# facebookresearch/multipathnet

Hardware: NVIDIA H100
Metric: proposals/sec (higher is better)
Workload: dtype fp32 (wgmma split emulation, fp32 accumulate: 3 bf16 products per MAC, 2 fp16 products in fc6/fc7)

## Files before the change

multipathnet_b200/csrc/gemm_tc.cu:

```cuda
#include "conv_gemm.cuh"
#include "wgmma.cuh"
#include "fp8_e4m3.cuh"
#include <algorithm>
#include <stdlib.h>
#include <string.h>

namespace {

constexpr int BM = 128;
constexpr int BK = 64;
constexpr int TC_THREADS = 384;
constexpr int CONS_THREADS = 256;
constexpr int A_TILE_BYTES = BM * BK * 2;
constexpr int SMEM_BUDGET = 196608;

__host__ __device__ constexpr int a_planes(OperandScheme ops) { return (ops == OperandScheme::BF16X1 || ops == OperandScheme::FP8X1) ? 1 : 2; }
__host__ __device__ constexpr int b_planes(OperandScheme ops) { return ops == OperandScheme::BF16X3 ? 2 : 1; }
__host__ __device__ constexpr int elem_bytes(OperandScheme ops) { return ops == OperandScheme::FP8X1 ? 1 : 2; }
__host__ __device__ constexpr int row_bytes(int BN, OperandScheme ops) { return (ops == OperandScheme::FP8X1 || BN == 256) ? 64 : 128; }
__host__ __device__ constexpr int stage_k(int BN, OperandScheme ops) { return row_bytes(BN, ops) / elem_bytes(ops); }
__host__ __device__ constexpr int kb_steps(int BN, OperandScheme ops) { return BK / stage_k(BN, ops); }
__host__ __device__ constexpr int a_tile_bytes(int BN, OperandScheme ops) { return BM * row_bytes(BN, ops); }
__host__ __device__ constexpr int stage_bytes(int BN, OperandScheme ops = OperandScheme::BF16X3) {
  return (a_planes(ops) * BM + b_planes(ops) * BN) * row_bytes(BN, ops);
}
__host__ __device__ constexpr int max_stages(int BN, OperandScheme ops) { return row_bytes(BN, ops) == 64 ? 8 : 4; }
__host__ __device__ constexpr int num_stages(int BN, OperandScheme ops = OperandScheme::BF16X3) {
  return (SMEM_BUDGET / stage_bytes(BN, ops)) > max_stages(BN, ops) ? max_stages(BN, ops) : (SMEM_BUDGET / stage_bytes(BN, ops));
}
constexpr int EPI_WARP_BYTES = 16 * 128;
constexpr int EPI_BYTES = (CONS_THREADS / 32) * EPI_WARP_BYTES;
__host__ __device__ constexpr int tc_smem_bytes(int BN, OperandScheme ops) {
  return num_stages(BN, ops) * stage_bytes(BN, ops) + EPI_BYTES + 1024  + 256 ;
}

struct TcParams {
  int N, Ho, Wo, Cout;
  int kh, kw, stride, pad;
  int cblocks;
  int tn, th, tw;
  int tiles_img, tiles_h, tiles_w, tiles_n;
  int units;
  const float *bias;
  const __nv_bfloat16 *res_hi, *res_lo; long long res_ld;
  __nv_bfloat16 *out_hi, *out_lo; long long out_ld;
  float *out_f32; long long out_f32_ld;
  __nv_bfloat16 *pool_hi, *pool_lo; long long pool_ld; int Hp, Wp;
  int relu;
  int splitk, kb_per_split;
  long long split_stride;
  unsigned long long *tl_min, *tl_max;
  float acc_scale;
  int out_fmt;
  unsigned *ovf;
  const int *a_exp, *b_exp; long long sample_pix;
};

__device__ __forceinline__ unsigned long long gtimer() {
  unsigned long long t; asm volatile("mov.u64 %0, %%globaltimer;" : "=l"(t)); return t;
}
__device__ __forceinline__ void tl_min_stamp(const unsigned long long *base_, int i) {
  if (base_) atomicMin(const_cast<unsigned long long *>(base_) + i, gtimer());
}
__device__ __forceinline__ void tl_max_stamp(const unsigned long long *base_, int i) {
  if (base_) atomicMax(const_cast<unsigned long long *>(base_) + i, gtimer());
}
__device__ __forceinline__ uint32_t smem_u32(const void *p) { return (uint32_t)__cvta_generic_to_shared(p); }
__device__ __forceinline__ void mbar_init(uint32_t bar, uint32_t count) {
  asm volatile("mbarrier.init.shared::cta.b64 [%0], %1;" ::"r"(bar), "r"(count) : "memory");
}
__device__ __forceinline__ void mbar_expect_tx(uint32_t bar, uint32_t bytes) {
  asm volatile("mbarrier.arrive.expect_tx.shared::cta.b64 _, [%0], %1;" ::"r"(bar), "r"(bytes) : "memory");
}
__device__ __forceinline__ void mbar_arrive(uint32_t bar) {
  asm volatile("mbarrier.arrive.shared::cta.b64 _, [%0];" ::"r"(bar) : "memory");
}
__device__ __forceinline__ void mbar_wait(uint32_t bar, uint32_t parity) {
  uint32_t done;
  uint32_t spins = 0;
  do {
    asm volatile(
        "{\n\t.reg .pred p;\n\t"
        "mbarrier.try_wait.parity.shared::cta.b64 p, [%1], %2;\n\t"
        "selp.u32 %0, 1, 0, p;\n\t}"
        : "=r"(done) : "r"(bar), "r"(parity) : "memory");
    if (!done && ++spins == (1u << 26)) __trap();
  } while (!done);
}
__device__ __forceinline__ void tma_load_4d(uint32_t dst, const CUtensorMap *tm, uint32_t bar, int c0, int c1,
                                            int c2, int c3) {
  asm volatile(
      "cp.async.bulk.tensor.4d.shared::cluster.global.mbarrier::complete_tx::bytes [%0], [%1, {%3, %4, %5, %6}], [%2];"
      ::"r"(dst), "l"(reinterpret_cast<uint64_t>(tm)), "r"(bar), "r"(c0), "r"(c1), "r"(c2), "r"(c3) : "memory");
}
__device__ __forceinline__ void tma_load_2d(uint32_t dst, const CUtensorMap *tm, uint32_t bar, int c0, int c1) {
  asm volatile(
      "cp.async.bulk.tensor.2d.shared::cluster.global.mbarrier::complete_tx::bytes [%0], [%1, {%3, %4}], [%2];"
      ::"r"(dst), "l"(reinterpret_cast<uint64_t>(tm)), "r"(bar), "r"(c0), "r"(c1) : "memory");
}
__device__ __forceinline__ void prefetch_tmap(const CUtensorMap *tm) {
  asm volatile("prefetch.tensormap [%0];" ::"l"(reinterpret_cast<uint64_t>(tm)) : "memory");
}

__device__ __forceinline__ uint64_t make_smem_desc(uint32_t saddr) {
  uint64_t d = 0;
  d |= (uint64_t)((saddr & 0x3FFFFu) >> 4);
  d |= (uint64_t)1 << 16;
  d |= (uint64_t)(1024 >> 4) << 32;
  d |= (uint64_t)1 << 62;
  return d;
}

__device__ __forceinline__ uint64_t make_smem_desc_64b(uint32_t saddr) {
  uint64_t d = 0;
  d |= (uint64_t)((saddr & 0x3FFFFu) >> 4);
  d |= (uint64_t)1 << 16;
// ... 97 lines not shown
      float b[2] = {0.f, 0.f};
      int eb[2] = {0, 0};
#pragma unroll
      for (int k = 0; k < 2; ++k) {
        if (p.bias && c + k < p.Cout) b[k] = __ldg(p.bias + c + k);
        if constexpr (OPS == OperandScheme::FP8X1) eb[k] = __ldg(p.b_exp + c + k);
      }
#pragma unroll
      for (int i = 0; i < 2; ++i) {
        float &f0 = f[4 * j + 2 * i], &f1 = f[4 * j + 2 * i + 1];
        if constexpr (OPS == OperandScheme::FP16X2) { f0 *= p.acc_scale; f1 *= p.acc_scale; }
        if constexpr (OPS == OperandScheme::FP8X1) {
          f0 *= mpn_fp8::pow2(-(ea[i] + eb[0])); f1 *= mpn_fp8::pow2(-(ea[i] + eb[1]));
        }
        if (p.bias) {
          if (c < p.Cout) f0 += b[0];
          if (c + 1 < p.Cout) f1 += b[1];
        }
        if (p.res_hi && full8 && fok[i]) {
          const float2 x = bf16x2_to_float2(*reinterpret_cast<const uint32_t *>(p.res_hi + fpix[i] * p.res_ld + c));
          const float2 y = bf16x2_to_float2(*reinterpret_cast<const uint32_t *>(p.res_lo + fpix[i] * p.res_ld + c));
          f0 += x.x + y.x; f1 += x.y + y.y;
        }
        if (p.relu) { f0 = fmaxf(f0, 0.f); f1 = fmaxf(f1, 0.f); }
        if (out_f32 && fok[i]) {
          float *o = out_f32 + fpix[i] * p.out_f32_ld + c;
          if (c < p.Cout) o[0] = f0;
          if (c + 1 < p.Cout) o[1] = f1;
        }
      }
    }
    float mx[16];
    if (pool) {
#pragma unroll
      for (int j = 0; j < 8; ++j)
#pragma unroll
        for (int k = 0; k < 2; ++k) {
          float top = fok[0] ? f[4 * j + k] : -INFINITY, bot = fok[1] ? f[4 * j + 2 + k] : -INFINITY;
          top = fmaxf(top, __shfl_xor_sync(0xffffffffu, top, 4));
          bot = fmaxf(bot, __shfl_xor_sync(0xffffffffu, bot, 4));
          mx[2 * j + k] = fmaxf(top, bot);
        }
    }
#pragma unroll 1
    for (int plane = 0; plane < 2; ++plane) {
      if (p.out_hi) {
        uint32_t v[16];
#pragma unroll
        for (int j = 0; j < 8; ++j)
#pragma unroll
          for (int i = 0; i < 2; ++i) {
            uint32_t hi2 = 0, lo2 = 0;
            if (fok[i]) split_x2(p.out_fmt, f[4 * j + 2 * i], f[4 * j + 2 * i + 1], hi2, lo2, p.ovf);
            v[8 * i + j] = plane ? lo2 : hi2;
          }
        store_plane_chunk(so, v, plane ? p.out_lo : p.out_hi, p.out_ld, p, u, rbase, col0, lane);
      }
      if (pool) {
        const int pr = lane >> 3;
        __syncwarp();
        if (!(lane & 4) && fok[0]) {
#pragma unroll
          for (int j = 0; j < 8; ++j) {
            uint32_t hi2, lo2;
            split_x2(p.out_fmt, mx[2 * j], mx[2 * j + 1], hi2, lo2, p.ovf);
            const uint32_t a = so + (uint32_t)(pr * 128 + ((j ^ pr) * 16) + 4 * (lane & 3));
            asm volatile("st.shared.b32 [%0], %1;" ::"r"(a), "r"(plane ? lo2 : hi2) : "memory");
          }
        }
        __syncwarp();
        const int ch = lane & 7;
        uint4 d;
        asm volatile("ld.shared.v4.b32 {%0, %1, %2, %3}, [%4];" : "=r"(d.x), "=r"(d.y), "=r"(d.z), "=r"(d.w)
                     : "r"(so + (uint32_t)(pr * 128 + ((ch ^ pr) * 16))) : "memory");
        if (pok && col0 + 8 * ch < p.Cout)
          *reinterpret_cast<uint4 *>((plane ? p.pool_lo : p.pool_hi) + ppix * p.pool_ld + col0 + 8 * ch) = d;
      }
    }
#pragma unroll
    for (int k = 0; k + 32 < BN / 2; ++k) acc[k] = acc[k + 32];
  }
}

template <int BN, OperandScheme OPS = OperandScheme::BF16X3>
__global__ void __launch_bounds__(TC_THREADS, 1)
conv_gemm_tc_kernel(const __grid_constant__ CUtensorMap tmA_hi, const __grid_constant__ CUtensorMap tmA_lo,
                    const __grid_constant__ CUtensorMap tmB_hi, const __grid_constant__ CUtensorMap tmB_lo,
                    const TcParams p) {
  constexpr int S = num_stages(BN, OPS);
  constexpr int STAGE = stage_bytes(BN, OPS);
  constexpr int A_TILE = a_tile_bytes(BN, OPS);
  constexpr int B_TILE_BYTES = BN * row_bytes(BN, OPS);
  constexpr int B_OFF = a_planes(OPS) * A_TILE;
  constexpr int KSTEPS = kb_steps(BN, OPS);
  static_assert(S >= 2 && 2 * S * 8 <= 256, "ring depth: at least two stages, barriers in their 256 bytes");
  extern __shared__ uint8_t smem_raw[];
  uint8_t *smem = reinterpret_cast<uint8_t *>((reinterpret_cast<uintptr_t>(smem_raw) + 1023) & ~(uintptr_t)1023);
  uint64_t *bars = reinterpret_cast<uint64_t *>(smem + (size_t)S * STAGE + EPI_BYTES);
  const uint32_t smem_base = smem_u32(smem);
  const uint32_t bar_base = smem_u32(bars);
  auto full_bar = [&](int s) { return bar_base + 8u * s; };
  auto empty_bar = [&](int s) { return bar_base + 8u * (S + s); };

  const int tid = threadIdx.x, lane = tid & 31;
  const int num_kb = p.kh * p.kw * p.cblocks;

  if (tid == 0) {
    tl_min_stamp(p.tl_min, 0);
    if (a_planes(OPS) == 1) { prefetch_tmap(&tmA_hi); prefetch_tmap(&tmB_hi); }
    else { prefetch_tmap(&tmA_hi); prefetch_tmap(&tmA_lo); prefetch_tmap(&tmB_hi); prefetch_tmap(&tmB_lo); }
    for (int s = 0; s < S; ++s) { mbar_init(full_bar(s), 1); mbar_init(empty_bar(s), CONS_THREADS / 32); }
    asm volatile("fence.mbarrier_init.release.cluster;" ::: "memory");
  }
  __syncthreads();
  asm volatile("griddepcontrol.wait;" ::: "memory");
  asm volatile("griddepcontrol.launch_dependents;" ::: "memory");
  if (tid == 0) tl_min_stamp(p.tl_min, 1);

  if (tid < 128) {
    asm volatile("setmaxnreg.dec.sync.aligned.u32 24;" ::: "memory");
    if (tid == 0) {
      int it = 0;
      for (int unit = (int)blockIdx.x; unit < p.units; unit += (int)gridDim.x) {
        const UnitPos u = unit_pos(p, unit);
        const int kb0 = u.split * p.kb_per_split, kb1 = min(num_kb, kb0 + p.kb_per_split);
        const int w_in0 = u.twi * p.tw * p.stride - p.pad, h_in0 = u.thi * p.th * p.stride - p.pad, n0 = u.tni * p.tn;
        const int b_row0 = u.nt * BN;
        for (int kb = kb0; kb < kb1; ++kb) {
          const int tap = kb / p.cblocks, cb = kb - tap * p.cblocks;
          const int khi = tap / p.kw, kwi = tap - khi * p.kw;
#pragma unroll
          for (int h = 0; h < KSTEPS; ++h, ++it) {
            const int s = it % S; const uint32_t ph = (uint32_t)(it / S) & 1u;
            const int ka = cb * BK + h * stage_k(BN, OPS), kk = kb * BK + h * stage_k(BN, OPS);
            mbar_wait(empty_bar(s), ph ^ 1u);
            const uint32_t sa = smem_base + (uint32_t)s * STAGE;
            mbar_expect_tx(full_bar(s), (uint32_t)STAGE);
            tma_load_4d(sa, &tmA_hi, full_bar(s), ka, w_in0 + kwi, h_in0 + khi, n0);
            if (a_planes(OPS) == 2) tma_load_4d(sa + A_TILE, &tmA_lo, full_bar(s), ka, w_in0 + kwi, h_in0 + khi, n0);
            tma_load_2d(sa + B_OFF, &tmB_hi, full_bar(s), kk, b_row0);
            if (b_planes(OPS) == 2) tma_load_2d(sa + B_OFF + B_TILE_BYTES, &tmB_lo, full_bar(s), kk, b_row0);
          }
        }
      }
    }
    return;
  }

  asm volatile("setmaxnreg.inc.sync.aligned.u32 240;" ::: "memory");
  const int e = tid - 128;
  const int g = e >> 7, wq = (e >> 5) & 3;
  const uint32_t so = smem_base + (uint32_t)(S * STAGE + (e >> 5) * EPI_WARP_BYTES);
  int it = 0;
  for (int unit = (int)blockIdx.x; unit < p.units; unit += (int)gridDim.x) {
    const UnitPos u = unit_pos(p, unit);
    const int kb0 = u.split * p.kb_per_split, kb1 = min(num_kb, kb0 + p.kb_per_split);
    float acc[BN / 2];
#pragma unroll
    for (int i = 0; i < BN / 2; ++i) acc[i] = 0.f;
    if constexpr (OPS == OperandScheme::FP8X1) {
      float part[BN / 2];
#pragma unroll
      for (int i = 0; i < BN / 2; ++i) part[i] = 0.f;
      for (int kb = kb0; kb < kb1; ++kb, ++it) {
        const int s = it % S; const uint32_t ph = (uint32_t)(it / S) & 1u;
        mbar_wait(full_bar(s), ph);
        if (it == 0 && e == 0) tl_min_stamp(p.tl_min, 2);
        const uint32_t sa = smem_base + (uint32_t)s * STAGE;
        const uint64_t a8 = make_smem_desc_64b(sa + (uint32_t)g * (A_TILE / 2));
        const uint64_t b8 = make_smem_desc_64b(sa + B_OFF);
#pragma unroll
        for (int k = 0; k < BK / 32; ++k) {
          wgmma_fence_acc(part);
          wgmma_fence();
          wgmma_e4m3_nk32<BN>(part, a8 + (uint64_t)(2 * k), b8 + (uint64_t)(2 * k), 0u);
          wgmma_commit();
          wgmma_wait<0>();
          wgmma_fence_acc(part);
#pragma unroll
          for (int i = 0; i < BN / 2; ++i) acc[i] += part[i];
        }
        if (lane == 0) mbar_arrive(empty_bar(s));
      }
    } else {
      const int steps = (kb1 - kb0) * KSTEPS;
      for (int i = 0; i < steps; ++i, ++it) {
        const int s = it % S; const uint32_t ph = (uint32_t)(it / S) & 1u;
        mbar_wait(full_bar(s), ph);
        if (it == 0 && e == 0) tl_min_stamp(p.tl_min, 2);
        const uint32_t sa = smem_base + (uint32_t)s * STAGE;
        auto desc = [](uint32_t a) { return row_bytes(BN, OPS) == 64 ? make_smem_desc_64b(a) : make_smem_desc(a); };
        const uint64_t a_hi = desc(sa + (uint32_t)g * (A_TILE / 2));
        const uint64_t a_lo = desc(sa + A_TILE + (uint32_t)g * (A_TILE / 2));
        const uint64_t b_hi = desc(sa + B_OFF);
        const uint64_t b_lo = desc(sa + B_OFF + B_TILE_BYTES);
        wgmma_fence_acc(acc);
        wgmma_fence();
        mma_kstep<BN, OPS>(acc, a_hi, a_lo, b_hi, b_lo, i == 0);
        wgmma_commit();
        wgmma_wait<1>();
        wgmma_fence_acc(acc);
        if (i > 0 && lane == 0) mbar_arrive(empty_bar((it - 1) % S));
      }
      wgmma_wait<0>();
      wgmma_fence_acc(acc);
      if (lane == 0) mbar_arrive(empty_bar((it - 1) % S));
    }
    if (e == 0) tl_max_stamp(p.tl_max, 0);
    const uint32_t t_epi = (p.tl_max && e == 0) ? (uint32_t)gtimer() : 0u;
    tile_epilogue<BN, OPS>(p, u, acc, g, wq, lane, so);
    if (e == 0) {
      tl_max_stamp(p.tl_max, 1);
      if (p.tl_max) atomicAdd(p.tl_max + 3, (unsigned long long)((uint32_t)gtimer() - t_epi));
    }
  }
}


constexpr int C1_THREADS = 256;
constexpr int C1_A_BYTES = 2 * A_TILE_BYTES;
constexpr int C1_B_BYTES = 2 * 64 * 128;
constexpr int C1_OUT_WARP = 16 * 128;
constexpr int C1_SMEM = 2 * C1_A_BYTES + C1_B_BYTES + (C1_THREADS / 32) * C1_OUT_WARP + 1024;

__device__ __forceinline__ void conv1_gather(const float *__restrict__ x, int pix, int pixels, int H, int W, int bhalf,
                                             float (&in)[16]) {
#pragma unroll
  for (int k = 0; k < 16; ++k) in[k] = 0.f;
  if (pix < pixels) {
    const int HW = H * W;
    const int n = pix / HW, rem = pix - n * HW;
    const int ho = rem / W, wo = rem - ho * W;
    const float *x0 = x + ((size_t)n * 3 * HW + (size_t)(ho - 1) * W + (wo - 1));
    const bool rok[3] = {ho >= 1, true, ho + 1 < H}, cok[3] = {wo >= 1, true, wo + 1 < W};
#pragma unroll
    for (int k = 0; k < 16; ++k) {
      const int kk = 16 * bhalf + k;
      if (kk < 27) {
        const int ci = kk / 9, r = (kk / 3) % 3, q = kk % 3;
        in[k] = (rok[r] && cok[q]) ? __ldg(x0 + ci * HW + r * W + q) : 0.f;
      }
    }
  }
// ... 97 lines not shown
      for (int h = 0; h < 2; ++h) {
        float &f0 = acc[4 * j + 2 * h], &f1 = acc[4 * j + 2 * h + 1];
        f0 += b.x; f1 += b.y;
        if (relu) { f0 = fmaxf(f0, 0.f); f1 = fmaxf(f1, 0.f); }
      }
    }
    const int pix0 = tile * BM + 64 * g + 16 * (warp & 3);
#pragma unroll 1
    for (int plane = 0; plane < 2; ++plane) {
      uint32_t v[16];
#pragma unroll
      for (int j = 0; j < 8; ++j)
#pragma unroll
        for (int h = 0; h < 2; ++h) {
          uint32_t hi2, lo2;
          split_bf16x2(acc[4 * j + 2 * h], acc[4 * j + 2 * h + 1], hi2, lo2);
          v[8 * h + j] = plane ? lo2 : hi2;
        }
      conv1_store_plane(so, v, plane ? out_lo : out_hi, pix0, pixels, lane);
    }
  }
}

struct ReduceParams {
  const float *ws; long long split_stride; int splitk; long long pixels; int Cout;
  const float *bias; const __nv_bfloat16 *res_hi, *res_lo; long long res_ld; int relu;
  __nv_bfloat16 *out_hi, *out_lo; long long out_ld; float *out_f32; long long out_f32_ld;
  OutScatter scatter;
};
__global__ void __launch_bounds__(256) splitk_reduce_kernel(const ReduceParams r) {
  MPN_PDL_SYNC();
  const long long idx = (long long)blockIdx.x * blockDim.x + threadIdx.x;
  if (idx >= r.pixels * r.Cout) return;
  const long long pix = idx / r.Cout; const int c = (int)(idx - pix * r.Cout);
  float acc = 0.f;
  for (int s = 0; s < r.splitk; ++s) acc += r.ws[(long long)s * r.split_stride + idx];
  if (r.bias) acc += __ldg(r.bias + c);
  if (r.res_hi) acc += join_bf16(r.res_hi[pix * r.res_ld + c], r.res_lo[pix * r.res_ld + c]);
  if (r.relu) acc = fmaxf(acc, 0.f);
  if (r.out_hi) { __nv_bfloat16 h, l; split_bf16(acc, h, l); r.out_hi[pix * r.out_ld + c] = h; r.out_lo[pix * r.out_ld + c] = l; }
  if (r.scatter.n > 0) {
#pragma unroll 1
    for (int g = 0; g < r.scatter.n; ++g)
      if (c >= r.scatter.seg[g].c0 && c < r.scatter.seg[g].c1) { r.scatter.seg[g].ptr[pix * r.scatter.seg[g].ld + (c - r.scatter.seg[g].c0)] = acc; break; }
  } else if (r.out_f32) r.out_f32[pix * r.out_f32_ld + c] = acc;
}

typedef CUresult (*PFN_encodeTiled)(CUtensorMap *, CUtensorMapDataType, cuuint32_t, void *, const cuuint64_t *,
                                    const cuuint64_t *, const cuuint32_t *, const cuuint32_t *, CUtensorMapInterleave,
                                    CUtensorMapSwizzle, CUtensorMapL2promotion, CUtensorMapFloatOOBfill);
PFN_encodeTiled get_encode_fn() {
  static PFN_encodeTiled fn = nullptr;
  if (!fn) {
    void *p = nullptr; cudaDriverEntryPointQueryResult q;
    if (cudaGetDriverEntryPoint("cuTensorMapEncodeTiled", &p, cudaEnableDefault, &q) == cudaSuccess &&
        q == cudaDriverEntryPointSuccess)
      fn = reinterpret_cast<PFN_encodeTiled>(p);
  }
  return fn;
}

int encode_map(mpn_ctx *ctx, CUtensorMap *tm, const void *base, int rank, const cuuint64_t *dims,
               const cuuint64_t *strides_bytes , const cuuint32_t *box, const cuuint32_t *estr, int BN, OperandScheme ops) {
  const bool fp8 = ops == OperandScheme::FP8X1;
  PFN_encodeTiled fn = get_encode_fn();
  if (!fn) return mpn_fail(ctx, MPN_ERR_CUDA, "cuTensorMapEncodeTiled entry point unavailable");
  CUresult r = fn(tm, fp8 ? CU_TENSOR_MAP_DATA_TYPE_UINT8 : CU_TENSOR_MAP_DATA_TYPE_BFLOAT16, (cuuint32_t)rank, const_cast<void *>(base), dims,
                  strides_bytes, box, estr, CU_TENSOR_MAP_INTERLEAVE_NONE, row_bytes(BN, ops) == 64 ? CU_TENSOR_MAP_SWIZZLE_64B : CU_TENSOR_MAP_SWIZZLE_128B,
                  CU_TENSOR_MAP_L2_PROMOTION_L2_256B, CU_TENSOR_MAP_FLOAT_OOB_FILL_NONE);
  if (r != CUDA_SUCCESS) {
    char b[256];
    snprintf(b, sizeof b, "cuTensorMapEncodeTiled failed (%d): rank %d dims %llu %llu box %u %u", (int)r, rank,
             (unsigned long long)dims[0], (unsigned long long)dims[1], box[0], box[1]);
    return mpn_fail(ctx, MPN_ERR_CUDA, b);
  }
  return MPN_OK;
}

inline bool tc_use_pdl() {
  static const int on = [] { const char *e = getenv("MPN_TC_PDL"); return (e && e[0] == '0') ? 0 : 1; }();
  return on != 0;
}

template <int BN, OperandScheme OPS = OperandScheme::BF16X3>
int launch_bn(mpn_ctx *ctx, const ConvPlan &pl, const TcParams &tp) {
  const int smem = tc_smem_bytes(BN, OPS);
  constexpr int bslot = BN == 256 ? 2 : (BN == 128 ? 1 : 0);
  constexpr int slot = OPS == OperandScheme::FP16X2 ? 3 : (OPS == OperandScheme::BF16X1 ? 5 + bslot
                                                         : (OPS == OperandScheme::FP8X1 ? 8 + bslot : bslot));
  if (!ctx->tc_attr_set[slot]) {
    MPN_CUDA(ctx, cudaFuncSetAttribute(conv_gemm_tc_kernel<BN, OPS>, cudaFuncAttributeMaxDynamicSharedMemorySize, smem));
    ctx->tc_attr_set[slot] = 1;
  }
  const long long units = (long long)pl.tiles_img * pl.tiles_h * pl.tiles_w * pl.tiles_n * pl.splitk;
  MPN_CHECK_ARG(ctx, units > 0 && units < (1ll << 31), "conv_tc: grid size out of range");
  TcParams tpu = tp;
  tpu.units = (int)units;
  cudaLaunchConfig_t cfg = {};
  cfg.gridDim = dim3((unsigned)std::min<long long>(units, ctx->sm_count));
  cfg.blockDim = dim3(TC_THREADS); cfg.dynamicSmemBytes = (size_t)smem; cfg.stream = ctx->stream;
  cudaLaunchAttribute attr[1];
  int na = 0;
  if (tc_use_pdl()) {
    attr[na].id = cudaLaunchAttributeProgrammaticStreamSerialization;
    attr[na].val.programmaticStreamSerializationAllowed = 1;
    ++na;
  }
  cfg.attrs = attr; cfg.numAttrs = na;
  MPN_CUDA(ctx, cudaLaunchKernelEx(&cfg, conv_gemm_tc_kernel<BN, OPS>, pl.tmA_hi, pl.tmA_lo, pl.tmB_hi, pl.tmB_lo, tpu));
  MPN_LAUNCHED(ctx);
  return MPN_OK;
}

int launch_ops(mpn_ctx *ctx, const ConvPlan &pl, const TcParams &tp) {
  if (pl.ops == OperandScheme::FP16X2) return launch_bn<256, OperandScheme::FP16X2>(ctx, pl, tp);
  if (pl.ops == OperandScheme::FP8X1)
    return pl.BN == 128 ? launch_bn<128, OperandScheme::FP8X1>(ctx, pl, tp) : launch_bn<64, OperandScheme::FP8X1>(ctx, pl, tp);
  if (pl.ops == OperandScheme::BF16X1) {
    switch (pl.BN) {
      case 256: return launch_bn<256, OperandScheme::BF16X1>(ctx, pl, tp);
      case 128: return launch_bn<128, OperandScheme::BF16X1>(ctx, pl, tp);
      default: return launch_bn<64, OperandScheme::BF16X1>(ctx, pl, tp);
    }
  }
  switch (pl.BN) {
    case 256: return launch_bn<256>(ctx, pl, tp);
    case 128: return launch_bn<128>(ctx, pl, tp);
    default: return launch_bn<64>(ctx, pl, tp);
  }
}

}

int conv1_tc_launch(mpn_ctx *ctx, const float *x_nchw, int N, int H, int W, const float *w_dev, const float *bias_dev, int relu,
                    DTensor &y) {
  MPN_CHECK_ARG(ctx, y.hi && y.lo && y.C == 64 && y.ld % 8 == 0, "conv1_tc: output must be 64-channel split planes");
  MPN_CHECK_ARG(ctx, bias_dev, "conv1_tc: bias missing");
  MPN_CHECK_ARG(ctx, y.ld == 64 && (long long)N * H * W < (1ll << 31) - 256, "conv1_tc: dense 64-channel output and < 2^31 pixels");
  if (!ctx->tc_attr_set[4]) {
    MPN_CUDA(ctx, cudaFuncSetAttribute(conv1_tc_kernel, cudaFuncAttributeMaxDynamicSharedMemorySize, C1_SMEM));
    ctx->tc_attr_set[4] = 1;
  }
  const long long tiles = ((long long)N * H * W + BM - 1) / BM;
  cudaLaunchConfig_t cfg = {};
  cfg.gridDim = dim3((unsigned)std::min<long long>(tiles, 2ll * ctx->sm_count)); cfg.blockDim = dim3(C1_THREADS);
  cfg.dynamicSmemBytes = (size_t)C1_SMEM; cfg.stream = ctx->stream;
  cudaLaunchAttribute attr[1];
  int na = 0;
  if (tc_use_pdl()) { attr[na].id = cudaLaunchAttributeProgrammaticStreamSerialization; attr[na].val.programmaticStreamSerializationAllowed = 1; ++na; }
  cfg.attrs = attr; cfg.numAttrs = na;
  MPN_CUDA(ctx, cudaLaunchKernelEx(&cfg, conv1_tc_kernel, x_nchw, N, H, W, w_dev, bias_dev, relu, y.hi, y.lo));
  MPN_LAUNCHED(ctx);
  return MPN_OK;
}

double conv_flops(const ConvProblem &p) {
  const double Ho = (double)p.y.H, Wo = (double)p.y.W;
  return 2.0 * (double)p.x.C * p.Cout * p.kh * p.kw * Ho * Wo * (double)p.y.N;
}

static int conv_tc_plan_impl(mpn_ctx *ctx, int sm_count, const ConvProblem &p, ConvPlan &pl, bool choose_only) {
  pl.valid = 0;
  MPN_CHECK_ARG(ctx, choose_only || (p.x.hi && (p.x.lo || p.bf16) && ((p.w_hi && (p.w_lo || p.bf16)) || p.w16)),
                "conv_tc: operands must be split-bf16 (or an fp16 weight plane)");
  MPN_CHECK_ARG(ctx, !(p.w16 && p.bf16), "conv_tc: the bf16 numerics do not take an fp16 weight plane");
  MPN_CHECK_ARG(ctx, !(p.fp8 && (p.w16 || p.bf16)), "conv_tc: the fp8 numerics take neither an fp16 weight plane nor the bf16 numerics");
  MPN_CHECK_ARG(ctx, choose_only || !p.fp8 || (p.x8 && p.x8_exp && p.w8 && p.w8_exp), "conv_tc: the fp8 numerics need e4m3 planes and exponents");
  pl.ops = p.w16 ? OperandScheme::FP16X2 : (p.fp8 ? OperandScheme::FP8X1 : (p.bf16 ? OperandScheme::BF16X1 : OperandScheme::BF16X3));
  const bool w16 = pl.ops == OperandScheme::FP16X2, fp8 = pl.ops == OperandScheme::FP8X1;
  MPN_CHECK_ARG(ctx, choose_only || (p.x.fmt == 1) == w16, "conv_tc: fp16 activation planes go with the fp16 weight plane (and only with it)");
  MPN_CHECK_ARG(ctx, p.x.C % 8 == 0, "conv_tc: Cin must be a multiple of 8");
  MPN_CHECK_ARG(ctx, !fp8 || p.x.C % BK == 0, "conv_tc: the fp8 numerics need Cin a multiple of 64 (their quantizer groups are 64 channels wide)");
  MPN_CHECK_ARG(ctx, !w16 || p.x.C % BK == 0, "conv_tc: the fp16-weight path needs Cin a multiple of 64");
  const int cblocks = (int)(conv_k_pad(p.x.C) / BK);
  MPN_CHECK_ARG(ctx, p.x.ld % 8 == 0, "conv_tc: input pixel stride must be a multiple of 8 elements");
  MPN_CHECK_ARG(ctx, p.stride >= 1 && p.stride <= 2, "conv_tc: stride must be 1 or 2");
  const int Ho = (int)p.y.H, Wo = (int)p.y.W, N = (int)p.y.N;
  pl.flat = (p.kh == 1 && p.kw == 1 && p.stride == 1 && p.pad == 0) ? 1 : 0;
  pl.mode = 0; pl.splitk = 1;
  cuuint64_t dims[4], strides[3]; cuuint32_t box[4], estr[4];
  int gtn = 1, gth = 1, gtw = BM;
  if (!pl.flat) {
    double best = -1.0;
    for (int tw = 1; tw <= 128; tw <<= 1)
      for (int th = 1; th * tw <= 128; th <<= 1) {
        const int tn = 128 / (tw * th);
        if (tw * p.stride > 256 || th * p.stride > 256) continue;
        const long long tiles = (long long)((Wo + tw - 1) / tw) * ((Ho + th - 1) / th) * ((N + tn - 1) / tn);
        const double util = (double)N * Ho * Wo / (double)(tiles * 128) + 1e-6 * tw;
        if (util > best) { best = util; gtn = tn; gth = th; gtw = tw; }
      }
  }
  const long long P = (long long)p.x.N * p.x.H * p.x.W;
  {
    const bool r3_ok = (p.kh == 3 && p.kw == 3 && p.stride == 1 && p.pad == 1);
    const char *env3 = getenv("MPN_TC_R3");
    const char *env3m = getenv("MPN_TC_R3_MINPIX");
    const long long r3_minpix = env3m ? atoll(env3m) : 0;
    pl.mode = (r3_ok && !(env3 && env3[0] == '0') && P >= r3_minpix) ? 1 : 0;
  }
  const long long tiles_m = pl.flat ? (P + BM - 1) / BM
                                    : (pl.mode ? (long long)((Wo + 7) / 8) * ((Ho + 15) / 16) * N
                                               : (long long)((Wo + gtw - 1) / gtw) * ((Ho + gth - 1) / gth) * ((N + gtn - 1) / gtn));
  {
    const int taps = p.kh * p.kw;
    const double kblocks = (double)taps * (double)cblocks;
    double best = 1e300; int best_bn = 64;
    for (int bi = 0; bi < 3; ++bi) {
      const int bn = bi == 0 ? 256 : (bi == 1 ? 128 : 64);
      if (w16 && bn != 256) continue;
      if (fp8 && bn == 256) continue;
      if (!p.m_invariant && bn > 64 && bn > ((p.Cout + 63) / 64) * 64) continue;
      const int roi_bn = p.Cout > 128 ? 256 : (p.Cout > 64 ? 128 : 64);
      if (p.m_invariant && bn != (fp8 ? std::min(roi_bn, 128) : roi_bn)) continue;
      const long long units = tiles_m * ((p.Cout + bn - 1) / bn);
      const long long rounds = (units + sm_count - 1) / sm_count;
      const double mma = (w16 ? 2.0 : (pl.ops == OperandScheme::BF16X1 ? 1.0 : (fp8 ? 0.5 : 3.0))) * 128.0 * bn * 64.0 / 1024.0;
      const double ingest = ((double)a_planes(pl.ops) * 128 + (double)b_planes(pl.ops) * bn) * (fp8 ? 64.0 : 128.0) / 48.0;
      const double cost = (double)rounds * (kblocks * std::max(mma, ingest) + 1500.0 + 8.0 * bn);
      if (cost < best * 0.999) { best = cost; best_bn = bn; }
    }
    pl.BN = best_bn;
    pl.tiles_n = (p.Cout + pl.BN - 1) / pl.BN;
  }
  if (pl.flat) {
    pl.tn = 1; pl.th = 1; pl.tw = BM;
    pl.tiles_img = 1; pl.tiles_h = 1; pl.tiles_w = (int)((P + BM - 1) / BM);
    dims[0] = (cuuint64_t)p.x.C; dims[1] = (cuuint64_t)P; dims[2] = 1; dims[3] = 1;
    strides[0] = (cuuint64_t)p.x.ld * 2; strides[1] = (cuuint64_t)P * p.x.ld * 2; strides[2] = strides[1];
    box[0] = (cuuint32_t)stage_k(pl.BN, pl.ops); box[1] = BM; box[2] = 1; box[3] = 1;
    estr[0] = estr[1] = estr[2] = estr[3] = 1;
  } else {
    if (pl.mode == 1) { pl.tn = 1; pl.th = 16; pl.tw = 8; }
    else { pl.tn = gtn; pl.th = gth; pl.tw = gtw; }
    pl.tiles_w = (Wo + pl.tw - 1) / pl.tw; pl.tiles_h = (Ho + pl.th - 1) / pl.th; pl.tiles_img = (N + pl.tn - 1) / pl.tn;
    dims[0] = (cuuint64_t)p.x.C; dims[1] = (cuuint64_t)p.x.W; dims[2] = (cuuint64_t)p.x.H; dims[3] = (cuuint64_t)p.x.N;
    strides[0] = (cuuint64_t)p.x.ld * 2; strides[1] = (cuuint64_t)p.x.W * p.x.ld * 2;
    strides[2] = (cuuint64_t)p.x.H * p.x.W * p.x.ld * 2;
    box[0] = (cuuint32_t)stage_k(pl.BN, pl.ops); box[1] = (cuuint32_t)(pl.tw * p.stride); box[2] = (cuuint32_t)(pl.th * p.stride); box[3] = (cuuint32_t)pl.tn;
    estr[0] = 1; estr[1] = (cuuint32_t)p.stride; estr[2] = (cuuint32_t)p.stride; estr[3] = 1;
  }
  {
    const long long units = tiles_m * pl.tiles_n;
    const long long num_kb = (long long)p.kh * p.kw * cblocks;
    long long sk = std::min<long long>(num_kb / 8, 8);
    constexpr long long ROI_TILES_REF = 8;
    if (p.m_invariant && pl.flat && p.Cout <= 128) { if (sk < 2) sk = 1; }
    else if (p.m_invariant && pl.flat && p.fill_split)
      sk = std::max<long long>(1, std::min<long long>(sm_count / (ROI_TILES_REF * pl.tiles_n), num_kb / 8));
    else if (p.m_invariant) sk = 1;
    else if (p.wide_k_split && pl.flat && num_kb >= 256)
      sk = std::max<long long>({1, std::min<long long>(sm_count / units, num_kb / 8), (num_kb + 31) / 32});
    else if (pl.mode == 1 || sk < 2 || units * sk > sm_count) sk = 1;
    const char *env2 = getenv("MPN_TC_SPLITK");
    if (env2 && env2[0] == '0') sk = 1;
    pl.splitk = (int)std::max<long long>(sk, 1);
    pl.kb_per_split = (int)((num_kb + pl.splitk - 1) / pl.splitk);
    pl.splitk = (int)((num_kb + pl.kb_per_split - 1) / pl.kb_per_split);
  }
  if (choose_only) return MPN_OK;
  const long long Ktot = (long long)p.kh * p.kw * conv_k_pad(p.x.C);
  cuuint64_t bd[2] = {(cuuint64_t)Ktot, (cuuint64_t)p.Cout}, bs[1] = {(cuuint64_t)Ktot * 2};
  cuuint32_t bb[2] = {(cuuint32_t)stage_k(pl.BN, pl.ops), (cuuint32_t)pl.BN}, be[2] = {1, 1};
  if (fp8) {
    const cuuint64_t C8 = (cuuint64_t)p.x.C;
    if (pl.flat) { strides[0] = C8; strides[1] = (cuuint64_t)P * C8; strides[2] = strides[1]; }
    else { strides[0] = C8; strides[1] = (cuuint64_t)p.x.W * C8; strides[2] = (cuuint64_t)p.x.H * p.x.W * C8; }
    bs[0] = (cuuint64_t)Ktot;
    MPN_TRY(encode_map(ctx, &pl.tmA_hi, p.x8, 4, dims, strides, box, estr, pl.BN, pl.ops));
    MPN_TRY(encode_map(ctx, &pl.tmB_hi, p.w8, 2, bd, bs, bb, be, pl.BN, pl.ops));
    pl.tmA_lo = pl.tmA_hi; pl.tmB_lo = pl.tmB_hi;
    pl.valid = 1;
    return MPN_OK;
  }
  MPN_TRY(encode_map(ctx, &pl.tmA_hi, p.x.hi, 4, dims, strides, box, estr, pl.BN, pl.ops));
  if (a_planes(pl.ops) == 2) { MPN_TRY(encode_map(ctx, &pl.tmA_lo, p.x.lo, 4, dims, strides, box, estr, pl.BN, pl.ops)); }
  else pl.tmA_lo = pl.tmA_hi;
  if (w16) {
    MPN_CHECK_ARG(ctx, pl.mode == 0 && pl.flat && pl.BN == 256, "conv_tc: the fp16-weight path is for wide flat GEMMs");
    MPN_TRY(encode_map(ctx, &pl.tmB_hi, p.w16, 2, bd, bs, bb, be, pl.BN, pl.ops));
    pl.tmB_lo = pl.tmB_hi;
  } else {
    MPN_TRY(encode_map(ctx, &pl.tmB_hi, p.w_hi, 2, bd, bs, bb, be, pl.BN, pl.ops));
    if (b_planes(pl.ops) == 2) { MPN_TRY(encode_map(ctx, &pl.tmB_lo, p.w_lo, 2, bd, bs, bb, be, pl.BN, pl.ops)); }
    else pl.tmB_lo = pl.tmB_hi;
  }
  pl.valid = 1;
  return MPN_OK;
}

int conv_tc_plan(mpn_ctx *ctx, const ConvProblem &p, ConvPlan &pl) { return conv_tc_plan_impl(ctx, ctx->sm_count, p, pl, false); }

int conv_tc_launch(mpn_ctx *ctx, const ConvProblem &p, const ConvPlan &pl) {
  MpnProfScope prof_scope__(ctx, MPN_CAT_CONV_TC);
  MPN_CHECK_ARG(ctx, pl.valid, "conv_tc_launch: invalid plan");
  TcParams tp;
  memset(&tp, 0, sizeof(tp));
  if (pl.flat) { tp.N = 1; tp.Ho = 1; tp.Wo = (int)(p.y.N * p.y.H * p.y.W); }
  else { tp.N = (int)p.y.N; tp.Ho = (int)p.y.H; tp.Wo = (int)p.y.W; }
  tp.Cout = p.Cout; tp.kh = p.kh; tp.kw = p.kw; tp.stride = p.stride; tp.pad = p.pad;
  tp.cblocks = (int)(conv_k_pad(p.x.C) / BK);
  tp.tn = pl.tn; tp.th = pl.th; tp.tw = pl.tw;
  tp.tiles_img = pl.tiles_img; tp.tiles_h = pl.tiles_h; tp.tiles_w = pl.tiles_w; tp.tiles_n = pl.tiles_n;
  tp.bias = p.bias;
  tp.res_hi = p.res.hi; tp.res_lo = p.res.lo; tp.res_ld = p.res.ld;
  tp.out_hi = p.y.hi; tp.out_lo = p.y.lo; tp.out_ld = p.y.ld;
  tp.out_f32 = p.y.f32; tp.out_f32_ld = p.y_f32_ld;
  tp.relu = p.relu;
  tp.splitk = pl.splitk; tp.kb_per_split = pl.kb_per_split; tp.split_stride = 0;
  tp.acc_scale = pl.ops == OperandScheme::FP16X2 ? p.w16_inv_scale : 1.f;
  tp.out_fmt = p.y.fmt; tp.ovf = nullptr;
  if (p.y.fmt) MPN_TRY(mpn_ovf_flag(ctx, &tp.ovf));
  if (pl.ops == OperandScheme::FP8X1) { tp.a_exp = p.x8_exp; tp.b_exp = p.w8_exp; tp.sample_pix = p.y.H * p.y.W; }
  MPN_CHECK_ARG(ctx, !p.pool.hi || p.pool.fmt == p.y.fmt, "conv_tc: pooled output must share the output's plane format");
  MPN_CHECK_ARG(ctx, !(p.y.fmt && pl.splitk > 1), "conv_tc: fp16 output planes are not written by the split-K reduce");
  MPN_CHECK_ARG(ctx, !p.res.hi || p.res.fmt == 0, "conv_tc: residual inputs are bf16 split planes");
  if (ctx->tl_on && ctx->tl_n < ctx->tl_cap) { tp.tl_min = ctx->tl_min + 4 * ctx->tl_n; tp.tl_max = ctx->tl_max + 4 * ctx->tl_n; ++ctx->tl_n; }
  if (p.pool.hi) {
    MPN_CHECK_ARG(ctx, pl.mode == 1 && pl.splitk == 1 && !p.res.hi && p.Cout % 8 == 0 && p.pool.ld % 8 == 0,
                  "conv_tc: fused pooling needs the 3x3 kernel, no residual, Cout multiple of 8");
    MPN_CHECK_ARG(ctx, p.pool.H == (p.y.H + 1) / 2 && p.pool.W == (p.y.W + 1) / 2 && p.pool.N == p.y.N, "conv_tc: pooled geometry mismatch");
    tp.pool_hi = p.pool.hi; tp.pool_lo = p.pool.lo; tp.pool_ld = p.pool.ld; tp.Hp = (int)p.pool.H; tp.Wp = (int)p.pool.W;
// ... 42 lines not shown
```

Measured before the change: 413,300.

## Add strip-reuse 3x3 conv path loading input strips once per column tap

Adds a STRIP variant of the TC conv kernel for mode-1 3x3 stride-1 plans with BN=64. It loads an 18-row input strip once per column tap and channel block, then reuses it across the three kernel rows by offsetting the smem descriptor, with separate A and B mbarrier rings. The aim is to cut redundant TMA input traffic, roughly a third of the A loads. In exchange it adds ring and barrier bookkeeping, a deeper weight ring, and a strict eligibility check that only small cblocks can satisfy.

```diff
diff --git a/multipathnet_b200/csrc/gemm_tc.cu b/multipathnet_b200/csrc/gemm_tc.cu
--- a/multipathnet_b200/csrc/gemm_tc.cu
+++ b/multipathnet_b200/csrc/gemm_tc.cu
@@ -32,6 +32,24 @@
 constexpr int EPI_BYTES = (CONS_THREADS / 32) * EPI_WARP_BYTES;
 __host__ __device__ constexpr int tc_smem_bytes(int BN, OperandScheme ops) {
   return num_stages(BN, ops) * stage_bytes(BN, ops) + EPI_BYTES + 1024  + 256 ;
+}
+
+constexpr int STRIP_ROWS = 18 * 8;
+constexpr int STRIP_BN = 64;
+__host__ __device__ constexpr bool strip_scheme(OperandScheme ops) { return ops == OperandScheme::BF16X3 || ops == OperandScheme::BF16X1; }
+__host__ __device__ constexpr int strip_plane_bytes(int BN, OperandScheme ops) { return STRIP_ROWS * row_bytes(BN, ops); }
+__host__ __device__ constexpr int strip_a_slot_bytes(int BN, OperandScheme ops) { return a_planes(ops) * strip_plane_bytes(BN, ops); }
+__host__ __device__ constexpr int strip_b_slot_bytes(int BN, OperandScheme ops) { return b_planes(ops) * BN * row_bytes(BN, ops); }
+__host__ __device__ constexpr int strip_slots_a(OperandScheme ops) { return ops == OperandScheme::BF16X3 ? 3 : 6; }
+__host__ __device__ constexpr int strip_slots_b(OperandScheme ops) { return ops == OperandScheme::BF16X3 ? 5 : 8; }
+__host__ __device__ constexpr bool strip_fits(int BN, OperandScheme ops, int cblocks) {
+  return BN == STRIP_BN && strip_scheme(ops) && 3 * cblocks * kb_steps(BN, ops) <= strip_slots_a(ops);
+}
+__host__ __device__ constexpr int strip_ring_bytes(int BN, OperandScheme ops) {
+  return strip_slots_a(ops) * strip_a_slot_bytes(BN, ops) + strip_slots_b(ops) * strip_b_slot_bytes(BN, ops);
+}
+__host__ __device__ constexpr int tc_smem_bytes(int BN, OperandScheme ops, bool strip) {
+  return strip ? strip_ring_bytes(BN, ops) + EPI_BYTES + 1024  + 256  : tc_smem_bytes(BN, ops);
 }
 
 struct TcParams {
@@ -295,7 +313,7 @@
   }
 }
 
-template <int BN, OperandScheme OPS = OperandScheme::BF16X3>
+template <int BN, OperandScheme OPS = OperandScheme::BF16X3, bool STRIP = false>
 __global__ void __launch_bounds__(TC_THREADS, 1)
 conv_gemm_tc_kernel(const __grid_constant__ CUtensorMap tmA_hi, const __grid_constant__ CUtensorMap tmA_lo,
                     const __grid_constant__ CUtensorMap tmB_hi, const __grid_constant__ CUtensorMap tmB_lo,
@@ -307,13 +325,24 @@
   constexpr int B_OFF = a_planes(OPS) * A_TILE;
   constexpr int KSTEPS = kb_steps(BN, OPS);
   static_assert(S >= 2 && 2 * S * 8 <= 256, "ring depth: at least two stages, barriers in their 256 bytes");
+  constexpr int SA = strip_slots_a(OPS), SB = strip_slots_b(OPS);
+  constexpr int A_SLOT = strip_a_slot_bytes(BN, OPS), B_SLOT = strip_b_slot_bytes(BN, OPS);
+  static_assert(!STRIP || (BN == STRIP_BN && strip_scheme(OPS) && SA >= 3 && SB >= 2 && 2 * (SA + SB) * 8 <= 256 &&
+                           strip_ring_bytes(BN, OPS) <= SMEM_BUDGET && A_SLOT % 1024 == 0 && B_SLOT % 1024 == 0),
+                "strip rings: a unit's strips for one channel block, two weight slots, barriers in their 256 bytes, within "
+                "the budget, atom-aligned slots");
+  constexpr int RING = STRIP ? strip_ring_bytes(BN, OPS) : S * STAGE;
   extern __shared__ uint8_t smem_raw[];
   uint8_t *smem = reinterpret_cast<uint8_t *>((reinterpret_cast<uintptr_t>(smem_raw) + 1023) & ~(uintptr_t)1023);
-  uint64_t *bars = reinterpret_cast<uint64_t *>(smem + (size_t)S * STAGE + EPI_BYTES);
+  uint64_t *bars = reinterpret_cast<uint64_t *>(smem + (size_t)RING + EPI_BYTES);
   const uint32_t smem_base = smem_u32(smem);
   const uint32_t bar_base = smem_u32(bars);
   auto full_bar = [&](int s) { return bar_base + 8u * s; };
   auto empty_bar = [&](int s) { return bar_base + 8u * (S + s); };
+  auto a_full = [&](int s) { return bar_base + 8u * s; };
+  auto a_empty = [&](int s) { return bar_base + 8u * (SA + s); };
+  auto b_full = [&](int s) { return bar_base + 8u * (2 * SA + s); };
+  auto b_empty = [&](int s) { return bar_base + 8u * (2 * SA + SB + s); };
 
   const int tid = threadIdx.x, lane = tid & 31;
   const int num_kb = p.kh * p.kw * p.cblocks;
@@ -322,7 +351,12 @@
     tl_min_stamp(p.tl_min, 0);
     if (a_planes(OPS) == 1) { prefetch_tmap(&tmA_hi); prefetch_tmap(&tmB_hi); }
     else { prefetch_tmap(&tmA_hi); prefetch_tmap(&tmA_lo); prefetch_tmap(&tmB_hi); prefetch_tmap(&tmB_lo); }
-    for (int s = 0; s < S; ++s) { mbar_init(full_bar(s), 1); mbar_init(empty_bar(s), CONS_THREADS / 32); }
+    if constexpr (STRIP) {
+      for (int s = 0; s < SA; ++s) { mbar_init(a_full(s), 1); mbar_init(a_empty(s), CONS_THREADS / 32); }
+      for (int s = 0; s < SB; ++s) { mbar_init(b_full(s), 1); mbar_init(b_empty(s), CONS_THREADS / 32); }
+    } else {
+      for (int s = 0; s < S; ++s) { mbar_init(full_bar(s), 1); mbar_init(empty_bar(s), CONS_THREADS / 32); }
+    }
     asm volatile("fence.mbarrier_init.release.cluster;" ::: "memory");
   }
   __syncthreads();
@@ -332,7 +366,37 @@
 
   if (tid < 128) {
     asm volatile("setmaxnreg.dec.sync.aligned.u32 24;" ::: "memory");
-    if (tid == 0) {
+    if (STRIP && tid == 0) {
+      int ia = 0, ib = 0;
+      for (int unit = (int)blockIdx.x; unit < p.units; unit += (int)gridDim.x) {
+        const UnitPos u = unit_pos(p, unit);
+        const int w_in0 = u.twi * p.tw - p.pad, h_in0 = u.thi * p.th - p.pad, n0 = u.tni * p.tn;
+        const int b_row0 = u.nt * BN;
+        for (int ky = 0; ky < 3; ++ky)
+          for (int kx = 0; kx < 3; ++kx)
+            for (int cb = 0; cb < p.cblocks; ++cb)
+#pragma unroll
+              for (int h = 0; h < KSTEPS; ++h, ++ib) {
+                if (ky == 0) {
+                  const int sa = ia % SA; const uint32_t pha = (uint32_t)(ia / SA) & 1u;
+                  const int ka = cb * BK + h * stage_k(BN, OPS);
+                  mbar_wait(a_empty(sa), pha ^ 1u);
+                  const uint32_t da = smem_base + (uint32_t)(sa * A_SLOT);
+                  mbar_expect_tx(a_full(sa), (uint32_t)A_SLOT);
+                  tma_load_4d(da, &tmA_hi, a_full(sa), ka, w_in0 + kx, h_in0, n0);
+                  if (a_planes(OPS) == 2) tma_load_4d(da + strip_plane_bytes(BN, OPS), &tmA_lo, a_full(sa), ka, w_in0 + kx, h_in0, n0);
+                  ++ia;
+                }
+                const int sb = ib % SB; const uint32_t phb = (uint32_t)(ib / SB) & 1u;
+                const int kk = ((ky * 3 + kx) * p.cblocks + cb) * BK + h * stage_k(BN, OPS);
+                mbar_wait(b_empty(sb), phb ^ 1u);
+                const uint32_t db = smem_base + (uint32_t)(SA * A_SLOT + sb * B_SLOT);
+                mbar_expect_tx(b_full(sb), (uint32_t)B_SLOT);
+                tma_load_2d(db, &tmB_hi, b_full(sb), kk, b_row0);
+                if (b_planes(OPS) == 2) tma_load_2d(db + B_TILE_BYTES, &tmB_lo, b_full(sb), kk, b_row0);
+              }
+      }
+    } else if (tid == 0) {
       int it = 0;
       for (int unit = (int)blockIdx.x; unit < p.units; unit += (int)gridDim.x) {
         const UnitPos u = unit_pos(p, unit);
@@ -363,15 +427,43 @@
   asm volatile("setmaxnreg.inc.sync.aligned.u32 240;" ::: "memory");
   const int e = tid - 128;
   const int g = e >> 7, wq = (e >> 5) & 3;
-  const uint32_t so = smem_base + (uint32_t)(S * STAGE + (e >> 5) * EPI_WARP_BYTES);
+  const uint32_t so = smem_base + (uint32_t)(RING + (e >> 5) * EPI_WARP_BYTES);
   int it = 0;
+  int ia = 0;
   for (int unit = (int)blockIdx.x; unit < p.units; unit += (int)gridDim.x) {
     const UnitPos u = unit_pos(p, unit);
     const int kb0 = u.split * p.kb_per_split, kb1 = min(num_kb, kb0 + p.kb_per_split);
     float acc[BN / 2];
 #pragma unroll
     for (int i = 0; i < BN / 2; ++i) acc[i] = 0.f;
-    if constexpr (OPS == OperandScheme::FP8X1) {
+    if constexpr (STRIP) {
+      auto desc = [](uint32_t a) { return row_bytes(BN, OPS) == 64 ? make_smem_desc_64b(a) : make_smem_desc(a); };
+      const int ns = 3 * p.cblocks * KSTEPS, steps = 3 * ns;
+      for (int i = 0, j = 0, ky = 0; i < steps; ++i, ++it) {
+        const int sa = (ia + j) % SA;
+        if (ky == 0) mbar_wait(a_full(sa), (uint32_t)((ia + j) / SA) & 1u);
+        const int sb = it % SB;
+        mbar_wait(b_full(sb), (uint32_t)(it / SB) & 1u);
+        if (it == 0 && e == 0) tl_min_stamp(p.tl_min, 2);
+        const uint32_t a_tap = smem_base + (uint32_t)(sa * A_SLOT + (8 * ky + 64 * g) * row_bytes(BN, OPS));
+        const uint32_t b = smem_base + (uint32_t)(SA * A_SLOT + sb * B_SLOT);
+        wgmma_fence_acc(acc);
+        wgmma_fence();
+        mma_kstep<BN, OPS>(acc, desc(a_tap), desc(a_tap + strip_plane_bytes(BN, OPS)), desc(b), desc(b + B_TILE_BYTES), i == 0);
+        wgmma_commit();
+        wgmma_wait<1>();
+        wgmma_fence_acc(acc);
+        if (i > 0 && lane == 0) {
+          mbar_arrive(b_empty((it - 1) % SB));
+          if (i > 2 * ns) mbar_arrive(a_empty((ia + j - 1) % SA));
+        }
+        if (++j == ns) { j = 0; ++ky; }
+      }
+      wgmma_wait<0>();
+      wgmma_fence_acc(acc);
+      if (lane == 0) { mbar_arrive(b_empty((it - 1) % SB)); mbar_arrive(a_empty((ia + ns - 1) % SA)); }
+      ia += ns;
+    } else if constexpr (OPS == OperandScheme::FP8X1) {
       float part[BN / 2];
 #pragma unroll
       for (int i = 0; i < BN / 2; ++i) part[i] = 0.f;
@@ -635,18 +727,23 @@
   return on != 0;
 }
 
-template <int BN, OperandScheme OPS = OperandScheme::BF16X3>
+template <int BN, OperandScheme OPS = OperandScheme::BF16X3, bool STRIP = false>
 int launch_bn(mpn_ctx *ctx, const ConvPlan &pl, const TcParams &tp) {
-  const int smem = tc_smem_bytes(BN, OPS);
+  const int smem = tc_smem_bytes(BN, OPS, STRIP);
   constexpr int bslot = BN == 256 ? 2 : (BN == 128 ? 1 : 0);
-  constexpr int slot = OPS == OperandScheme::FP16X2 ? 3 : (OPS == OperandScheme::BF16X1 ? 5 + bslot
-                                                         : (OPS == OperandScheme::FP8X1 ? 8 + bslot : bslot));
+  constexpr int slot = STRIP ? (OPS == OperandScheme::BF16X1 ? 11 : 10)
+                     : (OPS == OperandScheme::FP16X2 ? 3 : (OPS == OperandScheme::BF16X1 ? 5 + bslot
+                                                         : (OPS == OperandScheme::FP8X1 ? 8 + bslot : bslot)));
   if (!ctx->tc_attr_set[slot]) {
-    MPN_CUDA(ctx, cudaFuncSetAttribute(conv_gemm_tc_kernel<BN, OPS>, cudaFuncAttributeMaxDynamicSharedMemorySize, smem));
+    MPN_CUDA(ctx, cudaFuncSetAttribute(conv_gemm_tc_kernel<BN, OPS, STRIP>, cudaFuncAttributeMaxDynamicSharedMemorySize, smem));
     ctx->tc_attr_set[slot] = 1;
   }
   const long long units = (long long)pl.tiles_img * pl.tiles_h * pl.tiles_w * pl.tiles_n * pl.splitk;
   MPN_CHECK_ARG(ctx, units > 0 && units < (1ll << 31), "conv_tc: grid size out of range");
+  if (STRIP)
+    MPN_CHECK_ARG(ctx, pl.mode == 1 && pl.splitk == 1 && tp.kh == 3 && tp.kw == 3 && tp.stride == 1 && tp.pad == 1 &&
+                       tp.tn == 1 && tp.th == 16 && tp.tw == 8 && strip_fits(BN, OPS, tp.cblocks),
+                  "conv_tc: strip kernel needs a mode-1 plan without split-K whose strips fit its ring");
   TcParams tpu = tp;
   tpu.units = (int)units;
   cudaLaunchConfig_t cfg = {};
@@ -660,26 +757,29 @@
     ++na;
   }
   cfg.attrs = attr; cfg.numAttrs = na;
-  MPN_CUDA(ctx, cudaLaunchKernelEx(&cfg, conv_gemm_tc_kernel<BN, OPS>, pl.tmA_hi, pl.tmA_lo, pl.tmB_hi, pl.tmB_lo, tpu));
+  MPN_CUDA(ctx, cudaLaunchKernelEx(&cfg, conv_gemm_tc_kernel<BN, OPS, STRIP>, pl.tmA_hi, pl.tmA_lo, pl.tmB_hi, pl.tmB_lo, tpu));
   MPN_LAUNCHED(ctx);
   return MPN_OK;
 }
+
+inline bool plan_strip(const ConvPlan &pl, int cblocks) { return pl.mode == 1 && strip_fits(pl.BN, pl.ops, cblocks); }
 
 int launch_ops(mpn_ctx *ctx, const ConvPlan &pl, const TcParams &tp) {
   if (pl.ops == OperandScheme::FP16X2) return launch_bn<256, OperandScheme::FP16X2>(ctx, pl, tp);
   if (pl.ops == OperandScheme::FP8X1)
     return pl.BN == 128 ? launch_bn<128, OperandScheme::FP8X1>(ctx, pl, tp) : launch_bn<64, OperandScheme::FP8X1>(ctx, pl, tp);
+  const bool strip = plan_strip(pl, tp.cblocks);
   if (pl.ops == OperandScheme::BF16X1) {
     switch (pl.BN) {
       case 256: return launch_bn<256, OperandScheme::BF16X1>(ctx, pl, tp);
       case 128: return launch_bn<128, OperandScheme::BF16X1>(ctx, pl, tp);
-      default: return launch_bn<64, OperandScheme::BF16X1>(ctx, pl, tp);
+      default: return strip ? launch_bn<STRIP_BN, OperandScheme::BF16X1, true>(ctx, pl, tp) : launch_bn<64, OperandScheme::BF16X1>(ctx, pl, tp);
     }
   }
   switch (pl.BN) {
     case 256: return launch_bn<256>(ctx, pl, tp);
     case 128: return launch_bn<128>(ctx, pl, tp);
-    default: return launch_bn<64>(ctx, pl, tp);
+    default: return strip ? launch_bn<STRIP_BN, OperandScheme::BF16X3, true>(ctx, pl, tp) : launch_bn<64>(ctx, pl, tp);
   }
 }
 
@@ -791,6 +891,7 @@
     strides[0] = (cuuint64_t)p.x.ld * 2; strides[1] = (cuuint64_t)p.x.W * p.x.ld * 2;
     strides[2] = (cuuint64_t)p.x.H * p.x.W * p.x.ld * 2;
     box[0] = (cuuint32_t)stage_k(pl.BN, pl.ops); box[1] = (cuuint32_t)(pl.tw * p.stride); box[2] = (cuuint32_t)(pl.th * p.stride); box[3] = (cuuint32_t)pl.tn;
+    if (plan_strip(pl, cblocks)) box[2] = (cuuint32_t)(pl.th + 2);
     estr[0] = 1; estr[1] = (cuuint32_t)p.stride; estr[2] = (cuuint32_t)p.stride; estr[3] = 1;
   }
   {
```

After: 419,800 (median of 6 runs). 1.6% higher.
